# furiosa-ai/eta-inversion

Hardware: AMD Instinct MI355X
Metric: images/sec SD1.5 512^2 50-step etainv+ptp (higher is better)
Workload: dtype bf16; 1 GPU; etainv+ptp, SD1.5-shaped UNet (seeded synthetic weights), 512x512 (64x64 latents), 50 DDIM steps, 32 image pairs per GPU per step, eta [[0.6, 0], [1, 0.7]], n=10 noise candidates, cfg 7.5/1; images_per_gpu=32, unet_sample_forwards_per_image_reference=300

## Files before the change

### eta-inversion_amd/csrc/attention.hip

```cpp
#include <cstdlib>
#include <type_traits>

#include "common.h"
#include "kernels.h"
#include "self_attn_route.h"

namespace etainv {

template <typename T> struct Frag;
template <> struct Frag<f16> {
  typedef f16x8 v8;
  typedef f16x4 v4;
  static __device__ __forceinline__ f32x4 mfma(v8 a, v8 b, f32x4 c) { return __builtin_amdgcn_mfma_f32_16x16x32_f16(a, b, c, 0, 0, 0); }
};
template <> struct Frag<bf16> {
  typedef bf16x8 v8;
  typedef bf16x4 v4;
  static __device__ __forceinline__ f32x4 mfma(v8 a, v8 b, f32x4 c) { return __builtin_amdgcn_mfma_f32_16x16x32_bf16(a, b, c, 0, 0, 0); }
};

constexpr float NEG_BIG = -1.0e30f;

__device__ __forceinline__ void row_roles(int b, int n_img, int& half, int& role, int& img) {
  half = b / (2 * n_img);
// ... 657 lines not shown
        for (int qb = 0; qb < QB; ++qb) {
          v8 pf[4];
#pragma unroll
          for (int ks = 0; ks < 4; ++ks)
#pragma unroll
            for (int e = 0; e < 8; ++e) pf[ks][e] = (T)__builtin_amdgcn_exp2f(s[qb][ks >> 1][(ks & 1) * 8 + e]);
#pragma unroll
          for (int ks = 0; ks < 4; ++ks)
#pragma unroll
            for (int dt = 0; dt < DT; ++dt) o[qb][dt] = Frag32<T>::mfma(vf[ks][dt], pf[ks], o[qb][dt]);
        }
        if (j + 1 < ntiles) store_p(0, cur ^ 1);
        __syncthreads();
      }
    }

    const int q_base = qblk * QI + wid * (32 * QB);
#pragma unroll
    for (int qb = 0; qb < QB; ++qb) {
      const float l = __shfl(o[qb][GEO::LT][GEO::LI], r + 32 * GEO::LH, 64);
      const float inv = 1.f / l;
      const int query = q_base + qb * 32 + r;
      T* op = out + ((int64_t)b * N + query) * C + hd * D + 4 * h;
#pragma unroll
      for (int g4 = 0; g4 < D / 8; ++g4) {
        const int dt = g4 >> 2, i0 = (g4 & 3) * 4;
        T v[4] = {(T)(o[qb][dt][i0] * inv), (T)(o[qb][dt][i0 + 1] * inv), (T)(o[qb][dt][i0 + 2] * inv), (T)(o[qb][dt][i0 + 3] * inv)};
        *reinterpret_cast<u32x2*>(op + 8 * g4) = *reinterpret_cast<u32x2*>(v);
      }
    }
  }
}

template <typename T, int D, int QT, bool EDIT>
__global__ void __launch_bounds__(256) cross_attn_kernel(const T* __restrict__ q, const T* __restrict__ kv, T* __restrict__ out,
                                                         CrossParams p, int row0) {
  typedef typename Frag<T>::v8 v8;
  typedef typename Frag<T>::v4 v4;
  constexpr int DP = (D + 31) / 32 * 32;
  constexpr int KS = DP / 32;
  constexpr int DT = (D + 15) / 16;
  constexpr int NCH = D / 8;
  constexpr int KC = 96;
  constexpr int KT = 5;
  constexpr int KSTR = DP + 8;
  constexpr int VSTR = KC + 8;
  constexpr int PSTR = 81;

  extern __shared__ __attribute__((aligned(16))) char smem[];
  T* sK = reinterpret_cast<T*>(smem);
  T* sKs = sK + KC * KSTR;
  T* sVt = EDIT ? sKs + KC * KSTR : sKs;
  float* sP = reinterpret_cast<float*>(sVt + DT * 16 * VSTR);
  float* sTab = sP + 4 * QT * 16 * PSTR;

  const int tid = threadIdx.x, lane = tid & 63, wid = tid >> 6;
  const int fr = lane & 15, q4 = lane >> 4;
  int bx = blockIdx.x, gxn = gridDim.x, h = blockIdx.y, bz = blockIdx.z;
  if (p.xcd_gx > 0) {
    const int lin = blockIdx.x, xcd = lin & 7, t = lin >> 3;
    h = t % p.heads;
    const int c = (t / p.heads) * 8 + xcd;
    gxn = p.xcd_gx;
    bx = c % gxn;
    bz = c / gxn;
  }
  const int b = row0 + bz;
  const int N = p.N, C = p.heads * D, C2 = 2 * C;

  int img = 0, role = -1, is_cond = 0;
  if (p.layout == 2) {
    int half;
    row_roles(b + p.first_row, p.n_img, half, role, img);
    is_cond = half;
  } else if (p.layout == 1) {
    img = b % p.n_img;
    is_cond = (p.rows == p.n_img) ? 1 : (b / p.n_img);
    role = 0;
  } else if (p.layout == 3) {
    const int g = b / p.n_img;
    img = b % p.n_img;
    is_cond = g >= 1;
    role = g == 1 ? 1 : 0;
  }
  const bool do_edit = EDIT && p.edit && p.layout == 2 && is_cond && role == 1;
  const bool do_store = p.map_layer >= 0 && is_cond;
  const int bs = b - p.n_img;

  for (int idx = tid; idx < KC * (KSTR / 8); idx += 256) {
    const int key = idx / (KSTR / 8), ch = idx % (KSTR / 8);
    u32x4 a = {0u, 0u, 0u, 0u}, s = {0u, 0u, 0u, 0u};
    if (key < p.n_ctx && ch < NCH) {
      a = *reinterpret_cast<const u32x4*>(kv + ((int64_t)b * p.n_ctx + key) * C2 + h * D + ch * 8);
      if (do_edit) s = *reinterpret_cast<const u32x4*>(kv + ((int64_t)bs * p.n_ctx + key) * C2 + h * D + ch * 8);
    }
    *reinterpret_cast<u32x4*>(sK + key * KSTR + ch * 8) = a;
    if (EDIT) *reinterpret_cast<u32x4*>(sKs + key * KSTR + ch * 8) = s;
  }
  for (int idx = tid; idx < KC * NCH; idx += 256) {
    const int key = idx % KC, ch = idx / KC;
    u32x4 c = {0u, 0u, 0u, 0u};
    if (key < p.n_ctx) c = *reinterpret_cast<const u32x4*>(kv + ((int64_t)b * p.n_ctx + key) * C2 + C + h * D + ch * 8);
    const T* e = reinterpret_cast<const T*>(&c);
#pragma unroll
    for (int j = 0; j < 8; ++j) sVt[(ch * 8 + j) * VSTR + key] = e[j];
  }
  if (EDIT && do_edit && tid < p.n_ctx) {
    int mp = p.mapper ? p.mapper[img * 77 + tid] : 0;
    if (mp < 0) mp += p.n_ctx;
    sTab[0 * 80 + tid] = __builtin_bit_cast(float, mp);
    sTab[1 * 80 + tid] = p.alphas ? p.alphas[img * 77 + tid] : 0.f;
    sTab[2 * 80 + tid] = p.equalizer ? p.equalizer[img * 77 + tid] : 1.f;
    sTab[3 * 80 + tid] = p.cross_alpha[img * 77 + tid];
  }
  __syncthreads();

  constexpr bool QPF = D <= 80;
  u32x4 qn[QPF ? QT : 1][QPF ? 2 : 1][QPF ? KS : 1];
  auto load_q = [&](int qb, int qt, int brow, u32x4 (&dst)[QPF ? KS : 1]) __attribute__((always_inline)) {
    int query = qb * (64 * QT) + wid * (16 * QT) + qt * 16 + fr;
    query = query < N ? query : N - 1;
    const T* qp = q + ((int64_t)brow * N + query) * C + h * D;
#pragma unroll
    for (int ks = 0; ks < KS; ++ks) {
      const int d0 = ks * 32 + q4 * 8;
      u32x4 v = {0u, 0u, 0u, 0u};
      if (d0 < D) v = *reinterpret_cast<const u32x4*>(qp + d0);
      dst[ks] = v;
    }
  };
  auto load_block = [&](int qb) __attribute__((always_inline)) {
    if constexpr (QPF) {
#pragma unroll
      for (int qt = 0; qt < QT; ++qt) {
        load_q(qb, qt, b, qn[qt][0]);
        if (do_edit) load_q(qb, qt, bs, qn[qt][1]);
      }
    }
  };
  if (bx * (64 * QT) < N) load_block(bx);
  for (int qb = bx; qb * (64 * QT) < N; qb += gxn) {
  u32x4 qc[QPF ? QT : 1][QPF ? 2 : 1][QPF ? KS : 1];
  if constexpr (QPF) {
#pragma unroll
    for (int qt = 0; qt < QT; ++qt)
#pragma unroll
      for (int e = 0; e < 2; ++e)
#pragma unroll
        for (int ks = 0; ks < KS; ++ks) qc[qt][e][ks] = qn[qt][e][ks];
    if ((qb + gxn) * (64 * QT) < N) load_block(qb + gxn);
// ... 230 lines not shown
    CrossParams pl = p;
    dim3 grid(gx, p.heads, rows);
    if (xcd_heads && (gx * rows) % 8 == 0) {
      pl.xcd_gx = gx;
      grid = dim3(gx * p.heads * rows);
    }
    if (edit)
      hipLaunchKernelGGL((cross_attn_kernel<T, D, QT, true>), grid, dim3(256), lds_edit, s, (const T*)q, (const T*)kv, (T*)out, pl, row0);
    else
      hipLaunchKernelGGL((cross_attn_kernel<T, D, QT, false>), grid, dim3(256), lds_plain, s, (const T*)q, (const T*)kv, (T*)out, pl, row0);
  };
  if (p.edit && p.layout == 2) {
    const int edit0 = 3 * p.n_img - p.first_row;
    launch(false, 0, edit0);
    launch(true, edit0, b - edit0);
  } else {
    launch(false, 0, b);
  }
  ETAINV_LAUNCH_CHECK();
  return 0;
}

int launch_cross_attention_p(const void* q, const void* kv, void* out, int b, int d, const CrossParams& p, int dtype, hipStream_t s) {
  ETAINV_CHECK(q && kv && out && b > 0 && p.N > 0 && p.heads > 0, "bad arguments");
  ETAINV_CHECK(p.n_ctx >= 1 && p.n_ctx <= 77, "n_ctx must be in [1,77]");
  ETAINV_CHECK(d == 40 || d == 80 || d == 160, "head_dim must be 40, 80 or 160");
  ETAINV_CHECK(p.layout >= 0 && p.layout <= 3 && (p.layout == 0 || p.n_img >= 1), "cross-attention: layout 0..3, n_img >= 1");
  ETAINV_CHECK(p.layout != 1 || b == p.n_img || b == 2 * p.n_img, "cross-attention store layout [u, c] x n_img: n_img or 2*n_img rows");
  ETAINV_CHECK(p.layout != 2 || ((p.first_row == 0 || p.first_row == p.n_img) && b + p.first_row == 4 * p.n_img),
               "cross-attention prompt-to-prompt layout: rows [first_row, 4*n_img) of [u_s,u_t,c_s,c_t] x n_img, first_row 0 or n_img");
  ETAINV_CHECK(p.layout != 3 || b == 2 * p.n_img || b == 3 * p.n_img, "cross-attention layout [u_t, c_t, c_s] x n_img: 3*n_img rows, or 2*n_img once the source rows have left");
  ETAINV_CHECK(!p.edit || p.cross_alpha, "cross-attention edit without cross_alpha");
  ETAINV_CHECK(p.map_layer < 0 || (p.maps_acc && p.n_img <= p.n_img_cap), "cross-attention map store: maps_acc missing or n_img > n_img_cap");
  if (dtype == ETAINV_F32) return launch_cross_attention_f32(q, kv, out, b, d, p, s);
  ETAINV_DISPATCH_HALF(dtype, T, switch (d) {
    case 40: return launch_cross_t<T, 40>(q, kv, out, b, p, s);
    case 80: return launch_cross_t<T, 80>(q, kv, out, b, p, s);
    case 160: return launch_cross_t<T, 160>(q, kv, out, b, p, s);
    default: ETAINV_FAIL("head_dim must be 40, 80 or 160");
  });
  return 0;
}

}
```

### eta-inversion_amd/csrc/engine.cpp

```cpp
#include <cmath>
#include <cstring>
#include <functional>
#include <memory>
#include <string>
#include <unordered_map>
#include <vector>

#include "common.h"
#include "kernels.h"

namespace etainv {

static thread_local std::string g_err;
void set_error(const std::string& msg) { g_err = msg; }

struct ProfRec { int cls; double work, bytes; hipEvent_t a, b; };
static bool g_prof_on = false;
static std::vector<ProfRec> g_prof;
static std::vector<std::pair<hipEvent_t, hipEvent_t>> g_prof_pool;
static size_t g_prof_used = 0;
static bool g_prof_paused = false;
bool prof_enabled() { return g_prof_on && !g_prof_paused; }
void prof_pause(bool on) { g_prof_paused = on; }
void prof_begin(int cls, double work, hipStream_t s, double bytes) {
// ... 52 lines not shown

struct etainv_engine {
  etainv_engine_config cfg{};
  int dt = ETAINV_F16;
  size_t esz = 2;
  int L = 64, maxB = 4, max_img = 1;
  static constexpr int kHeads = 8, kCtx = 77, kCtxDim = 768, kGroups = 32, kTemb = 1280, kCh0 = 320;

  std::vector<WeightSlot> slots;
  std::unordered_map<std::string, int> slot_by_name;
  char* warena = nullptr;
  size_t wbytes = 0;
  char* wsarena = nullptr;
  size_t wsbytes = 0;

  void* conv_in_w = nullptr; float* conv_in_b = nullptr;
  void* conv_out_w = nullptr; float* conv_out_b = nullptr;
  Norm norm_out;
  Lin time1, time2, tproj;
  int tproj_total = 0;
  std::vector<ResBlock> res;
  std::vector<TBlock> tb;
  Lin down_conv[3], up_conv[3];

  void *skip[12] = {}, *tmp[3] = {}, *gnbuf = nullptr, *h1 = nullptr, *scbuf = nullptr;
  void *hsA = nullptr, *hsB = nullptr, *lnbuf = nullptr, *qkvbuf = nullptr, *attnbuf = nullptr, *qbuf = nullptr, *kvbuf = nullptr,
       *ffbuf = nullptr, *ctxT = nullptr, *tembuf = nullptr, *temb1 = nullptr, *temb2 = nullptr;
  float *tprojbuf = nullptr, *gn_scratch = nullptr, *maps_acc = nullptr, *lnstat = nullptr, *lnfinal = nullptr;
  size_t maps_bytes = 0;
  int map_div = 4, map_layers = 5;
  float *maps_alt = nullptr, *maps_cur = nullptr;
  size_t maps_alt_bytes = 0, maps_cur_bytes = 0;
  void* kvcache[16] = {};
  bool ctx_cache_on = false;
  const void* ctx_cached = nullptr;
  int ctx_rows = 0, ctx_io = -1;
  void* gn_bufs[16] = {};
  float* gn_part[16] = {};
  float* gn_final = nullptr;
  bool gn_fused = true;
  bool ln_fused = true;
  bool ln_folded = false;
  std::vector<hipStream_t> upload_streams;
  uint64_t ctx_gen = 0, ctx_gen_cached = 0;

  struct Tap { std::string name; int side = 1, channels = 0; void* dst = nullptr; int rows = 0; };
  std::vector<Tap> taps;
  int tap_index(const std::string& name) const {
    for (size_t i = 0; i < taps.size(); ++i)
      if (taps[i].name == name) return (int)i;
    return -1;
  }
  size_t tap_bytes(const Tap& t, int rows) const { return (size_t)rows * t.side * t.side * t.channels * esz; }

  long long qkv_hm_launches = 0;
  bool qkv_hm = true;
};

namespace {

struct ArenaPlan {
  size_t off = 0;
  size_t take(size_t bytes) {
    size_t o = off;
    off += (bytes + 255) & ~(size_t)255;
    return o;
// ... 230 lines not shown
    if (i < 3) {
      side *= 2;
      add(b + ".upsamplers.0", side, rev[i]);
    }
  }
  add("conv_norm_out", L, ch[0]);
}

int build_workspace(etainv_engine* e) {
  ArenaPlan plan;
  std::vector<std::function<void(char*)>> fix;
  auto want = [&](void** field, size_t bytes) {
    size_t off = plan.take(bytes);
    fix.push_back([field, off](char* base) { *field = base + off; });
  };
  const size_t B = (size_t)e->maxB, L = (size_t)e->L, esz = e->esz;
  const size_t hw[4] = {L * L, (L / 2) * (L / 2), (L / 4) * (L / 4), (L / 8) * (L / 8)};
  const size_t skip_el[12] = {hw[0] * 320, hw[0] * 320, hw[0] * 320, hw[1] * 320,  hw[1] * 640,  hw[1] * 640,
                              hw[2] * 640, hw[2] * 1280, hw[2] * 1280, hw[3] * 1280, hw[3] * 1280, hw[3] * 1280};
  for (int i = 0; i < 12; ++i) want(&e->skip[i], B * skip_el[i] * esz);
  const size_t hmax = hw[0] * 320;
  for (int i = 0; i < 3; ++i) want(&e->tmp[i], B * hw[0] * 640 * esz);
  want(&e->gnbuf, B * hw[0] * 960 * esz);
  want(&e->h1, B * hmax * esz);
  want(&e->scbuf, B * hmax * esz);
  want(&e->hsA, B * hmax * esz);
  want(&e->hsB, B * hmax * esz);
  want(&e->lnbuf, B * hmax * esz);
  want(&e->qkvbuf, B * hmax * 3 * esz);
  want(&e->attnbuf, B * hmax * esz);
  want(&e->qbuf, B * hmax * esz);
  want(&e->kvbuf, B * 77 * 2 * 1280 * esz);
  for (size_t i = 0; i < e->tb.size() && i < 16; ++i) want(&e->kvcache[i], B * 77 * 2 * (size_t)e->tb[i].c * esz);
  want(&e->ffbuf, B * hmax * 4 * esz);
  want(&e->ctxT, B * 77 * 768 * esz);
  want(&e->tembuf, B * 320 * esz);
  want(&e->temb1, B * 1280 * esz);
  want(&e->temb2, B * 1280 * esz);
  want(reinterpret_cast<void**>(&e->tprojbuf), B * (size_t)e->tproj_total * 4);
  want(reinterpret_cast<void**>(&e->gn_scratch), B * (GN_MAX_CHUNKS + 1) * etainv_engine::kGroups * 2 * 4);
  want(reinterpret_cast<void**>(&e->lnstat), B * hmax / 32 * 2 * 4);
  want(reinterpret_cast<void**>(&e->lnfinal), B * hw[0] * 2 * 4);
  for (int i = 0; i < 12; ++i) want(reinterpret_cast<void**>(&e->gn_part[i]), B * skip_el[i] / 16 * 4);
  for (int i = 0; i < 3; ++i) want(reinterpret_cast<void**>(&e->gn_part[12 + i]), B * hw[0] * 640 / 16 * 4);
  want(reinterpret_cast<void**>(&e->gn_part[15]), B * hmax / 16 * 4);
  want(reinterpret_cast<void**>(&e->gn_final), B * (etainv_engine::kGroups * 2 + 2 * 2560) * 4);
  const size_t res = L / 4;
  e->maps_bytes = (size_t)5 * e->max_img * 2 * etainv_engine::kHeads * res * res * 77 * 4;
  want(reinterpret_cast<void**>(&e->maps_acc), e->maps_bytes);
  e->wsbytes = plan.off;
  ETAINV_HIP(hipMalloc(reinterpret_cast<void**>(&e->wsarena), e->wsbytes));
  for (auto& f : fix) f(e->wsarena);
  for (int i = 0; i < 12; ++i) e->gn_bufs[i] = e->skip[i];
  for (int i = 0; i < 3; ++i) e->gn_bufs[12 + i] = e->tmp[i];
  e->gn_bufs[15] = e->h1;
  ETAINV_HIP(hipMemset(e->maps_acc, 0, e->maps_bytes));
  e->maps_cur = e->maps_acc;
  e->maps_cur_bytes = e->maps_bytes;
  return 0;
}

struct Fwd {
  etainv_engine* e;
  hipStream_t s;
  int rows;
  const etainv_attn_ctrl* ctrl;
// ... 130 lines not shown
    if (groupnorm(x, nullptr, c, 0, t.gn, hw, 1e-6f, 0)) return 1;
    if (run_ln_out(linear(e->gnbuf, t.proj_in, e->hsA, M))) return 1;
    int head_major = 0;
    IGemmParams qkv;
    if (ln_consumer(qkv, e->hsA, t.ln1, t.s_qkv, t.c_qkv, t.qkv, e->qkvbuf, M)) return 1;
    if (fold && e->qkv_hm && self_attn_prescaled_hm_ok(d, e->dt)) {
      IGemmParams hm = qkv;
      hm.hm_heads = etainv_engine::kHeads;
      hm.hm_dim = d;
      hm.hm_tokens = hw;
      if (igemm_hm_ok(hm, e->dt)) {
        head_major = 1;
        ++e->qkv_hm_launches;
        qkv = hm;
      }
    }
    if (run(qkv)) return 1;
    if (launch_self_attention_mode(e->qkvbuf, e->attnbuf, rows, hw, etainv_engine::kHeads, d, mode, n_img, e->dt, s, self_attn_prescaled_hm_ok(d, e->dt),
                                   ctrl ? (ctrl->src_exit_block ? -1 : ctrl->first_row) : 0, head_major)) return 1;
    IGemmParams o1 = linear(e->attnbuf, t.out1, e->hsB, M);
    o1.residual = e->hsA;
    if (run_ln_out(o1)) return 1;
    if (self_rows != all_rows) {
      const size_t off = (size_t)M * c * e->esz, Mn = (size_t)(all_rows - self_rows) * hw;
      ETAINV_HIP(hipMemcpyAsync(reinterpret_cast<char*>(e->hsB) + off, e->hsB, Mn * c * e->esz, hipMemcpyDeviceToDevice, s));
      if (fold) ETAINV_HIP(hipMemcpyAsync(e->lnfinal + (size_t)M * 2, e->lnfinal, Mn * 2 * sizeof(float), hipMemcpyDeviceToDevice, s));
      rows = all_rows;
      M = rows * hw;
    }
    IGemmParams q;
    if (ln_consumer(q, e->hsB, t.ln2, t.s_q, t.c_q, t.q, e->qbuf, M) || run(q)) return 1;
    void* kvb = e->kvcache[blk];
    if (!kv_reuse && run(linear(e->ctxT, t.kv, kvb, ctx_rows * etainv_engine::kCtx))) return 1;
    CrossParams cp;
    cp.N = hw;
    cp.heads = etainv_engine::kHeads;
    cp.n_ctx = etainv_engine::kCtx;
    cp.scale_log2 = (1.0f / std::sqrt((float)d)) * 1.4426950408889634f;
    cp.rows = rows;
    cp.n_img_cap = e->max_img;
    cp.maps_acc = e->maps_cur;
    cross_params_from_ctrl(cp, ctrl);
    if (cp.layout) {
      const int res = e->L / e->map_div;
      if (ctrl->store_maps && hw == res * res) {
        static const int layer_of_block[3][16] = {{-1, -1, 0, 1, -1, -1, -1, -1, -1, -1, 2, 3, 4, -1, -1, -1},
                                                  {-1, -1, -1, -1, 0, 1, -1, 2, 3, 4, -1, -1, -1, -1, -1, -1},
                                                  {-1, -1, -1, -1, -1, -1, 0, -1, -1, -1, -1, -1, -1, -1, -1, -1}};
        cp.map_layer = layer_of_block[e->map_div == 2 ? 0 : e->map_div == 4 ? 1 : 2][blk];
      }
    }
    if (launch_cross_attention_p(e->qbuf, kvb, e->attnbuf, rows, d, cp, e->dt, s)) return 1;
    IGemmParams o2 = linear(e->attnbuf, t.out2, e->hsA, M);
    o2.residual = e->hsB;
    if (run_ln_out(o2)) return 1;
    IGemmParams ff1;
    if (ln_consumer(ff1, e->hsA, t.ln3, t.s_ff1, t.c_ff1, t.ff1, e->ffbuf, M)) return 1;
    ff1.geglu = 1;
    if (run(ff1)) return 1;
    IGemmParams ff2 = linear(e->ffbuf, t.ff2, e->hsB, M);
    ff2.residual = e->hsA;
    if (run(ff2)) return 1;
    IGemmParams po = linear(e->hsB, t.proj_out, out, M);
    po.residual = x;
    return run(po, true);
  }
};

void* pick_tmp(etainv_engine* e, const void* a, const void* b) {
  for (int i = 0; i < 3; ++i)
    if (e->tmp[i] != a && e->tmp[i] != b) return e->tmp[i];
  return nullptr;
}

}

extern "C" int etainv_abi_version(void) { return ETAINV_ABI_VERSION; }
extern "C" const char* etainv_last_error(void) { return g_err.c_str(); }

extern "C" int etainv_engine_create(const etainv_engine_config* cfg, etainv_engine_t** out) {
  ETAINV_CHECK(cfg && out, "null argument");
  ETAINV_CHECK(cfg->compute_dtype == ETAINV_F16 || cfg->compute_dtype == ETAINV_BF16 || cfg->compute_dtype == ETAINV_F32, "compute_dtype must be f16, bf16 or f32");
  ETAINV_CHECK(cfg->latent_size >= 8 && cfg->latent_size % 8 == 0 && cfg->latent_size <= 128, "latent_size must be a multiple of 8 in [8,128]");
  ETAINV_CHECK(cfg->max_unet_batch >= 1 && cfg->max_img >= 1, "batch sizes must be positive");
  int ndev = 0;
  ETAINV_HIP(hipGetDeviceCount(&ndev));
  ETAINV_CHECK(ndev > 0, "no HIP device visible: the etainv engine has no CPU fallback");
  auto* e = new etainv_engine();
  e->cfg = *cfg;
  e->dt = cfg->compute_dtype;
  e->L = cfg->latent_size;
  e->maxB = cfg->max_unet_batch;
  e->max_img = cfg->max_img;
  e->esz = e->dt == ETAINV_F32 ? 4 : 2;
  e->ln_fused = !env_on("ETAINV_LN_UNFUSED") && e->dt != ETAINV_F32;
  e->gn_fused = !env_on("ETAINV_GN_UNFUSED") && e->dt != ETAINV_F32;
  e->qkv_hm = env_flag("ETAINV_QKV_HM", true);
  build_taps(e);
  if (build_model(e) || build_workspace(e)) {
    etainv_engine_destroy(e);
    return 1;
  }
  *out = e;
  return 0;
}

extern "C" int etainv_engine_destroy(etainv_engine_t* e) {
  if (!e) return 0;
  if (e->warena) (void)hipFree(e->warena);
  if (e->maps_alt) (void)hipFree(e->maps_alt);
  if (e->wsarena) (void)hipFree(e->wsarena);
  delete e;
  return 0;
}

extern "C" int etainv_engine_num_weights(etainv_engine_t* e) { return e ? (int)e->slots.size() : 0; }

extern "C" int etainv_engine_weight_info(etainv_engine_t* e, int i, char* name, int name_cap, int64_t shape[4], int* ndim) {
  ETAINV_CHECK(e && i >= 0 && i < (int)e->slots.size() && name && shape && ndim, "bad arguments");
  const WeightSlot& s = e->slots[i];
  ETAINV_CHECK((int)s.name.size() + 1 <= name_cap, "name buffer too small");
  std::memcpy(name, s.name.c_str(), s.name.size() + 1);
  for (int k = 0; k < 4; ++k) shape[k] = s.shape[k];
  *ndim = s.ndim;
  return 0;
}

extern "C" int etainv_engine_set_weight(etainv_engine_t* e, const char* name, const float* data, int64_t numel, void* stream) {
  ETAINV_CHECK(e && name && data, "null argument");
// ... 359 lines not shown
```

### eta-inversion_amd/csrc/kernels.h

```cpp
#pragma once
#include "common.h"

namespace etainv {

struct IGemmParams {
  const void* a1 = nullptr;
  const void* a2 = nullptr;
  const void* w = nullptr;
  const float* bias = nullptr;
  const float* rowvec = nullptr;
  int rowvec_stride = 0;
  int out_f32 = 0;
  int out_nchw = 0;
  int pad0 = 0;
  int out_io_dtype = 0;
  const void* residual = nullptr;
  void* out = nullptr;
  const void* zeros = nullptr;
  int debug = 0;
  int hm_heads = 0, hm_dim = 0, hm_tokens = 0, hm_magic = 0;
  unsigned long* stamps = nullptr;
  int M = 0, N = 0;
  int c1 = 0, c2 = 0;
  int H = 1, W = 1;
// ... 76 lines not shown
int launch_groupnorm(const void* x1, const void* x2, int c1, int c2, const float* gamma, const float* beta, void* out,
                     int b, int hw, int groups, float eps, int silu, float* scratch, int dtype, hipStream_t s);
int launch_groupnorm_pre(const void* x1, const void* x2, int c1, int c2, const float* part1, int wm1, const float* part2, int wm2, const float* gamma,
                         const float* beta, void* out, int b, int hw, int groups, float eps, int silu, float* final_stats, int dtype, hipStream_t s);
int launch_gn_finalize(int c1, int c2, const float* part1, int wm1, const float* part2, int wm2, int b, int hw, int groups, float eps, float* final_stats,
                       hipStream_t s, const float* gamma = nullptr, const float* beta = nullptr, float* scsh = nullptr);
int launch_gn_fold(const float* w, const float* gamma, const float* beta, const float* bias, const float* final_stats, int groups, int b, int n, int k,
                   void* wb_out, float* cb_out, int dtype, hipStream_t s);
int launch_layernorm(const void* x, const float* gamma, const float* beta, void* out, int rows, int c, float eps, int dtype,
                     hipStream_t s);
int launch_row_stats(const void* x, float* stat, int rows, int c, float eps, int dtype, hipStream_t s);
int launch_ln_finalize(const float* partials, int P, int cw, float eps, float* stat, int rows, hipStream_t s);

inline bool self_attn_prescaled_hm_ok(int d, int dtype) { return dtype != ETAINV_F32 && (d == 40 || d == 80); }
int launch_self_attention_mode(const void* qkv, void* out, int b, int n, int heads, int d, int mode, int n_img, int dtype,
                               hipStream_t s, int q_prescaled = 0, int first_row = 0, int head_major = 0);
struct CrossParams {
  int N = 0, heads = 8, n_ctx = 77;
  float scale_log2 = 0.f;
  int layout = 0;
  int n_img = 1;
  int rows = 0;
  int first_row = 0;
  int edit = 0;
  int map_layer = -1;
  int n_img_cap = 1;
  const int32_t* mapper = nullptr;
  const float* alphas = nullptr;
  const float* replace_mat = nullptr;
  const float* equalizer = nullptr;
  const float* cross_alpha = nullptr;
  float* maps_acc = nullptr;
  int xcd_gx = 0;
};
inline void cross_params_from_ctrl(CrossParams& cp, const etainv_attn_ctrl* ctrl) {
  if (!ctrl || (ctrl->mode != ETAINV_ATTN_PTP && ctrl->mode != ETAINV_ATTN_STORE)) return;
  const bool ptp = ctrl->mode == ETAINV_ATTN_PTP;
  cp.n_img = ctrl->n_img;
  cp.layout = ptp ? (ctrl->src_exit_block ? 3 : 2) : 1;
  cp.first_row = ptp ? ctrl->first_row : 0;
  if (ptp && (ctrl->mapper || ctrl->replace_mat)) {
    cp.edit = 1;
    cp.mapper = ctrl->mapper;
    cp.alphas = ctrl->alphas;
    cp.replace_mat = ctrl->replace_mat;
    cp.equalizer = ctrl->equalizer;
    cp.cross_alpha = ctrl->cross_alpha;
  }
}
int launch_cross_attention_p(const void* q, const void* kv, void* out, int b, int d, const CrossParams& p, int dtype, hipStream_t s);

int launch_im2col_in(const void* latent, int io_dtype, int n_lat, int rows, int L, void* out, int dtype, hipStream_t s);
int launch_time_embedding(const int64_t* t_host, int rows, int dim, void* out, int dtype, hipStream_t s);
int launch_silu(const void* x, void* out, int64_t n, int dtype, hipStream_t s);
enum PackMode { PK_PLAIN = 0, PK_CONV = 1, PK_GEGLU = 2, PK_CONV_IN_GEMM = 5 };
int launch_pack_ups4(const float* src, void* dst, int cout, int cin, int dtype, hipStream_t s);
int launch_pack_weight(const float* src, void* dst, int64_t rows, int64_t cols, int mode, int taps, int dtype, hipStream_t s, float scale = 1.0f,
                       const float* colscale = nullptr);
int launch_ln_fold(const float* w_src, const float* gamma, const float* beta, const float* bias_packed, int64_t rows, int64_t cols, int mode, float scale,
                   void* w_dst, float* s_dst, float* c_dst, int dtype, hipStream_t s);
int launch_cast_f32(const void* src, int src_dtype, void* dst, int dst_dtype, int64_t n, hipStream_t s);
int launch_rows_broadcast(void* x, int rows, int n_src, int64_t row_elems, int dtype, hipStream_t s);

int launch_prox_guidance(const float* eps_u, const float* eps_c, float g, int mode, int use_rank, int rank_lo, float rank_w, float thr_fixed,
                         float* eps_out, const float* x, float a_from, float a_to, float* x_out, float* thr_out, int n_groups, int rows_per_group,
                         int l, hipStream_t s);

// ... 11 lines not shown
```

### eta-inversion_amd/csrc/ops_capi.cpp

```cpp
#include <cmath>

#include "common.h"
#include "kernels.h"

using namespace etainv;

extern "C" int etainv_op_gemm(const void* a, const void* w, const void* bias, const void* residual, void* out, int m, int n, int k,
                              int geglu, int dtype, void* stream) {
  IGemmParams p = igemm_linear(a, w, (const float*)bias, out, m, n, k);
  p.residual = residual;
  p.geglu = geglu;
  return launch_igemm(p, dtype, (hipStream_t)stream);
}

extern "C" int etainv_op_gemm_ln(const void* a, const void* w_folded, const float* c_vec, const float* s_vec, const float* stat,
                                 const void* residual, void* out, float* stat_out, int* stat_p_out, int m, int n, int k, int geglu,
                                 int dtype, void* stream) {
  IGemmParams p = igemm_linear(a, w_folded, c_vec, out, m, n, k);
  p.residual = residual;
  p.geglu = geglu;
  if (stat) {
    p.ln_stat = stat;
    p.ln_s = s_vec;
  }
// ... 92 lines not shown
  p.taps = taps;
  return launch_igemm(p, dtype, (hipStream_t)stream);
}
extern "C" int etainv_op_conv3x3(const void* x_nhwc, const void* x2_nhwc, int c1, int c2, const void* w_okkc, const void* bias,
                                 const float* rowvec, const void* residual, void* out, int b, int h, int wd, int cout, int stride,
                                 int upsample, int taps, int dtype, void* stream) {
  return etainv_op_conv3x3_rv(x_nhwc, x2_nhwc, c1, c2, w_okkc, bias, rowvec, cout, residual, out, b, h, wd, cout, stride, upsample, taps, dtype, stream);
}

extern "C" int etainv_op_groupnorm(const void* x_nhwc, const void* x2_nhwc, int c1, int c2, const float* gamma, const float* beta,
                                   void* out, int b, int hw, int groups, float eps, int silu, float* scratch, int dtype, void* stream) {
  return launch_groupnorm(x_nhwc, x2_nhwc, c1, c2, gamma, beta, out, b, hw, groups, eps, silu, scratch, dtype, (hipStream_t)stream);
}

extern "C" int etainv_op_layernorm(const void* x, const float* gamma, const float* beta, void* out, int rows, int c, float eps, int dtype,
                                   void* stream) {
  return launch_layernorm(x, gamma, beta, out, rows, c, eps, dtype, (hipStream_t)stream);
}

extern "C" int etainv_op_self_attention(const void* qkv, void* out, int b, int n, int heads, int d, int mode, int n_img, int dtype,
                                        void* stream) {
  return launch_self_attention_mode(qkv, out, b, n, heads, d, mode, n_img, dtype, (hipStream_t)stream);
}

extern "C" int etainv_op_self_attention_ex(const void* qkv, void* out, int b, int n, int heads, int d, int mode, int n_img, int q_prescaled, int first_row,
                                           int head_major, int dtype, void* stream) {
  return launch_self_attention_mode(qkv, out, b, n, heads, d, mode, n_img, dtype, (hipStream_t)stream, q_prescaled, first_row, head_major);
}

extern "C" int etainv_op_rows_broadcast(void* x, int rows, int n_src, int64_t row_elems, int dtype, void* stream) {
  return launch_rows_broadcast(x, rows, n_src, row_elems, dtype, (hipStream_t)stream);
}

extern "C" int etainv_op_cross_attention(const void* q, const void* kv, void* out, int b, int n, int heads, int d, int n_ctx,
                                         const etainv_attn_ctrl* ctrl, int map_layer, int n_img_cap, float* maps_acc, int dtype,
                                         void* stream) {
  CrossParams cp;
  cp.N = n;
  cp.heads = heads;
  cp.n_ctx = n_ctx;
  cp.scale_log2 = (1.0f / std::sqrt((float)d)) * 1.4426950408889634f;
  cp.rows = b;
  cp.n_img_cap = n_img_cap;
  cp.maps_acc = maps_acc;
  cross_params_from_ctrl(cp, ctrl);
  if (cp.layout && ctrl->store_maps && map_layer >= 0) cp.map_layer = map_layer;
  return launch_cross_attention_p(q, kv, out, b, d, cp, dtype, (hipStream_t)stream);
}

extern "C" int etainv_op_gemm_f32out(const void* a, const void* w, const float* bias, float* out_f32, int m, int n, int k, int dtype, void* stream) {
  IGemmParams p = igemm_linear(a, w, bias, out_f32, m, n, k);
  p.out_f32 = 1;
  return launch_igemm(p, dtype, (hipStream_t)stream);
}

extern "C" int etainv_op_gn_fold(const float* w, const float* gamma, const float* beta, const float* bias, const float* stats, int groups, int b, int n,
                                 int k, void* wb_out, float* cb_out, int dtype, void* stream) {
  return launch_gn_fold(w, gamma, beta, bias, stats, groups, b, n, k, wb_out, cb_out, dtype, (hipStream_t)stream);
}

extern "C" int etainv_op_gemm_per_image(const void* a, const void* wb, const float* cb, const void* residual, void* out, int b, int hw, int n, int k,
                                        int dtype, void* stream) {
  ETAINV_CHECK(b > 0 && hw > 0, "bad sizes");
  IGemmParams p = igemm_linear(a, wb, cb, out, b * hw, n, k);
  p.residual = residual;
  p.rows_per_batch = hw;
  p.w_batch_stride = (int64_t)n * k;
  p.bias_batch_stride = n;
  return launch_igemm(p, dtype, (hipStream_t)stream);
}
// ... 55 lines not shown
```

### eta-inversion_amd/etainv/_capi.py

```python
import ctypes as C
import os
from pathlib import Path

F32, F16, BF16 = 0, 1, 2
ATTN_PLAIN, ATTN_STORE, ATTN_PTP, ATTN_MASA, ATTN_PNP = 0, 1, 2, 3, 4

_LIB_PATH = Path(__file__).resolve().parent / "lib" / "libetainv_hip.so"


class EtainvError(RuntimeError):
    pass


class EngineConfig(C.Structure):
    _fields_ = [("compute_dtype", C.c_int), ("max_unet_batch", C.c_int), ("latent_size", C.c_int), ("max_img", C.c_int),
                ("reserved", C.c_int * 4)]


class AttnCtrl(C.Structure):
    _fields_ = [("mode", C.c_int), ("n_img", C.c_int), ("store_maps", C.c_int),
                ("mapper", C.c_void_p), ("alphas", C.c_void_p), ("replace_mat", C.c_void_p), ("equalizer", C.c_void_p),
                ("cross_alpha", C.c_void_p),
                ("self_replace_active", C.c_int), ("self_max_tokens", C.c_int),
                ("masa_active", C.c_int), ("masa_first_block", C.c_int), ("first_row", C.c_int), ("src_exit_block", C.c_int), ("pnp_qk_active", C.c_int), ("pnp_conv_active", C.c_int)]
# ... 45 lines not shown
    "etainv_engine_tap_rows": [_p, _i],
    "etainv_engine_workspace_bytes": [_p],
    "etainv_engine_weight_bytes": [_p],
    "etainv_prof_enable": [_i],
    "etainv_prof_reset": [],
    "etainv_prof_read": [_i, C.POINTER(C.c_double), C.POINTER(C.c_double), C.POINTER(_i64)],
    "etainv_prof_records": [_i, C.POINTER(C.c_double), C.POINTER(C.c_double), _i64, C.POINTER(_i64)],
    "etainv_prof_records_ex": [_i, C.POINTER(C.c_double), C.POINTER(C.c_double), C.POINTER(C.c_double), _i64, C.POINTER(_i64)],
    "etainv_prof_split": [_i, C.c_double, C.POINTER(C.c_double), C.POINTER(_i64)],
    "etainv_op_gemm": [_p, _p, _p, _p, _p, _i, _i, _i, _i, _i, _p],
    "etainv_op_gemm_ln": [_p, _p, _p, _p, _p, _p, _p, _p, C.POINTER(_i), _i, _i, _i, _i, _i, _p],
    "etainv_op_gemm_ln_hm": [_p, _p, _p, _p, _p, _p, _i, _i, _i, _i, _i, _i, C.POINTER(_i), _i, _p],
    "etainv_engine_cache_context": [_p, _i],
    "etainv_engine_context_generation": [_p, C.c_uint64],
    "etainv_op_gemm_gnstat": [_p, _p, _p, _p, _p, _p, C.POINTER(_i), _i, _i, _i, _i, _i, _p],
    "etainv_op_conv3x3_gnstat": [_p, _p, _p, _p, _p, _p, _p, C.POINTER(_i), _i, _i, _i, _i, _i, _i, _p],
    "etainv_op_groupnorm_pre": [_p, _p, _i, _i, _p, _i, _p, _i, _p, _p, _p, _i, _i, _i, _f, _i, _p, _i, _p],
    "etainv_op_ln_fold": [_p, _p, _p, _p, _i, _i, _i, _f, _p, _p, _p, _i, _p],
    "etainv_op_row_stats": [_p, _p, _i, _i, _f, _i, _p],
    "etainv_op_ln_finalize": [_p, _i, _i, _f, _p, _i, _p],
    "etainv_op_pack_ups4": [_p, _p, _i, _i, _i, _p],
    "etainv_op_conv3x3": [_p, _p, _i, _i, _p, _p, _p, _p, _p, _i, _i, _i, _i, _i, _i, _i, _i, _p],
    "etainv_op_conv3x3_ex": [_p, _p, _p, _p, _p, _i, _i, _i, _i, _i, _i, _i, _i, _i, _i, _i, _p],
    "etainv_op_im2col3x3": [_p, _i, _i, _i, _i, _i, _p, _p, _i, _p],
    "etainv_op_row_softmax": [_p, _i, _i, _f, _i, _p],
    "etainv_op_quick_gelu": [_p, _p, _i64, _i, _p],
    "etainv_op_embed": [_p, _p, _p, _i, _i, _i, _p, _i, _p],
    "etainv_op_causal_attention": [_p, _p, _i, _i, _i, _i, _i, _p],
    "etainv_op_groupnorm": [_p, _p, _i, _i, _p, _p, _p, _i, _i, _i, _f, _i, _p, _i, _p],
    "etainv_op_layernorm": [_p, _p, _p, _p, _i, _i, _f, _i, _p],
    "etainv_op_self_attention": [_p, _p, _i, _i, _i, _i, _i, _i, _i, _p],
    "etainv_op_self_attention_ex": [_p, _p, _i, _i, _i, _i, _i, _i, _i, _i, _i, _i, _p],
    "etainv_op_cross_attention": [_p, _p, _p, _i, _i, _i, _i, _i, C.POINTER(AttnCtrl), _i, _i, _p, _i, _p],
    "etainv_op_word_maps": [_p, _i, _i, _i, _i, _i, _i, _p, _i, _i, _p, _i, _f, _p],
    "etainv_op_local_blend": [_p, _i, _i, _i, _i, _i, _p, _i, _p, _f, _p],
    "etainv_op_word_maps_ex": [_p, _i, _i, _i, _i, _i, _i, _p, _i, _i, _i, C.c_uint, _p, _i, _f, _p],
    "etainv_op_time_embedding": [C.POINTER(_i64), _i, _i, _p, _i, _p],
    "etainv_op_silu": [_p, _p, _i64, _i, _p],
    "etainv_op_cast": [_p, _i, _p, _i, _i64, _p],
    "etainv_op_im2col_in": [_p, _i, _i, _i, _i, _p, _i, _p],
    "etainv_op_pack_weight": [_p, _p, _i64, _i64, _i, _i, _f, _p, _i, _p],
    "etainv_op_gemm_f32out": [_p, _p, _p, _p, _i, _i, _i, _i, _p],
    "etainv_op_conv3x3_rv": [_p, _p, _i, _i, _p, _p, _p, _i, _p, _p, _i, _i, _i, _i, _i, _i, _i, _i, _p],
    "etainv_op_gn_fold": [_p, _p, _p, _p, _p, _i, _i, _i, _i, _p, _p, _i, _p],
    "etainv_op_gemm_per_image": [_p, _p, _p, _p, _p, _i, _i, _i, _i, _i, _p],
    "etainv_op_rows_broadcast": [_p, _i, _i, _i64, _i, _p],
    "etainv_op_last_igemm_plan": [C.POINTER(_i), _i],
    "etainv_op_igemm_route_name": [_i],
}
_RESTYPES = {"etainv_last_error": C.c_char_p, "etainv_op_igemm_route_name": C.c_char_p,"etainv_engine_workspace_bytes": _i64, "etainv_image_metrics_workspace_bytes": _i64, "etainv_engine_weight_bytes": _i64}

_lib = None


def lib_path() -> Path:
    return Path(os.environ.get("ETAINV_LIB", _LIB_PATH))


def load():
    global _lib
    if _lib is None:
        path = lib_path()
        if not path.exists():
            raise EtainvError(f"{path} not found: build it with eta-inversion_amd/csrc/build.sh (no CPU fallback exists)")
        lib = C.CDLL(str(path))
        for name, args in SIGNATURES.items():
            fn = getattr(lib, name)
            fn.argtypes = args
            fn.restype = _RESTYPES.get(name, C.c_int)
        _lib = lib
    return _lib


def check(status: int):
    if status != 0:
        raise EtainvError(load().etainv_last_error().decode())


def dtype_code(dt) -> int:
    import torch
    return {torch.float32: F32, torch.float16: F16, torch.bfloat16: BF16}[dt]


# ... 11 lines not shown
```

### include/etainv.h

```cpp
#ifndef ETAINV_H
#define ETAINV_H
#include <stdint.h>
#ifdef __cplusplus
extern "C" {
#endif

#define ETAINV_ABI_VERSION 1
#define ETAINV_MAX_WORDS 77

enum etainv_dtype { ETAINV_F32 = 0, ETAINV_F16 = 1, ETAINV_BF16 = 2 };

int etainv_abi_version(void);
const char* etainv_last_error(void);


int etainv_cfg_combine(const void* eps_u, const void* eps_c, float g, void* out, int64_t n,
                       int io_dtype, void* stream);

int etainv_ddim_step(const void* x, const void* eps, float a_from, float a_to, void* out, int64_t n,
                     int io_dtype, void* stream);

int etainv_ddim_eta_step(const void* x, const void* eps, float eta, const void* eta_mask, int n_mask, const void* noise,
                         float a_t, float a_p, float var, int rows, int c, int hw, void* out, int io_dtype, void* stream);

// ... 133 lines not shown
int etainv_op_gemm_gnstat(const void* a, const void* w, const float* bias, const void* residual, void* out, float* part, int* wm_out, int m,
                          int n, int k, int rows_per_image, int dtype, void* stream);
int etainv_op_conv3x3_gnstat(const void* x_nhwc, const void* w_okkc, const float* bias, const float* rowvec, const void* residual, void* out,
                             float* part, int* wm_out, int b, int h, int wd, int cin, int cout, int dtype, void* stream);
int etainv_op_groupnorm_pre(const void* x1, const void* x2, int c1, int c2, const float* part1, int wm1, const float* part2, int wm2,
                            const float* gamma, const float* beta, void* out, int b, int hw, int groups, float eps, int silu,
                            float* final_stats, int dtype, void* stream);
int etainv_op_pack_ups4(const float* w_oc33, void* dst, int cout, int cin, int dtype, void* stream);
int etainv_op_conv3x3(const void* x_nhwc, const void* x2_nhwc, int c1, int c2, const void* w_okkc, const void* bias,
                      const float* rowvec, const void* residual, void* out, int b, int h, int wd, int cout,
                      int stride, int upsample, int taps, int dtype, void* stream);
int etainv_op_conv3x3_ex(const void* x_nhwc, const void* w_okkc, const void* bias, const void* residual, void* out, int b, int h,
                         int wd, int cin, int cout, int stride, int upsample, int pad0, int out_nchw, int out_io_dtype, int dtype,
                         void* stream);
int etainv_op_im2col3x3(const void* x_nchw, int io_dtype, int cin, int h, int w, int rows, const float* premix, void* out,
                        int dtype, void* stream);
int etainv_op_row_softmax(void* x, int rows, int n, float scale, int dtype, void* stream);
int etainv_op_quick_gelu(const void* x, void* out, int64_t n, int dtype, void* stream);
int etainv_op_embed(const int64_t* ids, const void* tok, const void* pos, int b, int n_pos, int d, void* out, int dtype,
                    void* stream);
int etainv_op_causal_attention(const void* qkv, void* out, int b, int n, int heads, int d, int dtype, void* stream);
int etainv_op_groupnorm(const void* x_nhwc, const void* x2_nhwc, int c1, int c2, const float* gamma,
                        const float* beta, void* out, int b, int hw, int groups, float eps, int silu,
                        float* scratch, int dtype, void* stream);
int etainv_op_layernorm(const void* x, const float* gamma, const float* beta, void* out, int rows, int c,
                        float eps, int dtype, void* stream);
int etainv_op_self_attention(const void* qkv, void* out, int b, int n, int heads, int d, int mode, int n_img,
                             int dtype, void* stream);
int etainv_op_self_attention_ex(const void* qkv, void* out, int b, int n, int heads, int d, int mode, int n_img,
                                int q_prescaled, int first_row, int head_major, int dtype, void* stream);
int etainv_op_cross_attention(const void* q, const void* kv, void* out, int b, int n, int heads, int d,
                              int n_ctx, const etainv_attn_ctrl* ctrl, int map_layer, int n_img_cap,
                              float* maps_acc, int dtype, void* stream);
int etainv_op_word_maps(const float* maps_acc, int n_layers, int n_img_cap, int heads, int res, int L, int n_img,
                        const int32_t* tokens, int n_tok, int steps_done, float* out, int accumulate, float scale,
                        void* stream);
int etainv_op_local_blend(const float* maps_acc, int n_layers, int n_img_cap, int heads, int res, int L, float* x,
                          int n_img, const float* blend_alpha, float thres, void* stream);

int etainv_op_word_maps_ex(const float* maps_acc, int n_layers, int n_img_cap, int heads, int res, int L, int n_img,
                           const int32_t* tokens, int n_tok, int steps_done, int row_sel, unsigned layer_mask, float* out,
                           int accumulate, float scale, void* stream);
int etainv_op_time_embedding(const int64_t* t_host, int rows, int dim, void* out, int dtype, void* stream);
int etainv_op_silu(const void* x, void* out, int64_t n, int dtype, void* stream);
int etainv_op_cast(const void* src, int src_dtype, void* dst, int dst_dtype, int64_t n, void* stream);
int etainv_op_im2col_in(const void* latent, int io_dtype, int n_lat, int rows, int l, void* out, int dtype, void* stream);
int etainv_op_pack_weight(const float* src, void* dst, int64_t rows, int64_t cols, int mode, int taps, float scale, const float* colscale,
                          int dtype, void* stream);
int etainv_op_rows_broadcast(void* x, int rows, int n_src, int64_t row_elems, int dtype, void* stream);
int etainv_op_gemm_f32out(const void* a, const void* w, const float* bias, float* out_f32, int m, int n, int k, int dtype, void* stream);
int etainv_op_conv3x3_rv(const void* x_nhwc, const void* x2_nhwc, int c1, int c2, const void* w_okkc, const void* bias,
                         const float* rowvec, int rowvec_stride, const void* residual, void* out, int b, int h, int wd, int cout,
                         int stride, int upsample, int taps, int dtype, void* stream);
int etainv_op_gn_fold(const float* w, const float* gamma, const float* beta, const float* bias, const float* stats, int groups, int b, int n,
                      int k, void* wb_out, float* cb_out, int dtype, void* stream);
int etainv_op_gemm_per_image(const void* a, const void* wb, const float* cb, const void* residual, void* out, int b, int hw, int n, int k,
                             int dtype, void* stream);
int etainv_op_last_igemm_plan(int* out, int n);
const char* etainv_op_igemm_route_name(int route);

#ifdef __cplusplus
}
#endif
#endif
```

Measured before the change: 5.836 images/s.

## Precompute padded shared-memory K/V images for cross-attention once per context

Adds a kernel that writes each head's cross-attention K block and transposed V block into global memory, already padded in the exact shared-memory layout. It runs once whenever the context K/V projection is recomputed. Each cross-attention block then fills shared memory with straight vectorised copies instead of scattered transposing stores, and this cost is shared across the many query blocks of a head. It also turns on Q prefetch for the D=160 non-edit kernel. The price is extra workspace per transformer block and one extra kernel launch per K/V recompute.

New measurement: 5.846 images/s, median of 6. No clear change (+0.2%).

```diff
diff --git a/eta-inversion_amd/csrc/attention.hip b/eta-inversion_amd/csrc/attention.hip
--- a/eta-inversion_amd/csrc/attention.hip
+++ b/eta-inversion_amd/csrc/attention.hip
@@ -713,6 +713,36 @@
   }
 }
 
+template <typename T, int D>
+__global__ void __launch_bounds__(256) cross_kv_image_kernel(const T* __restrict__ kv, T* __restrict__ image, int heads, int n_ctx) {
+  constexpr int DP = (D + 31) / 32 * 32, DT = (D + 15) / 16, NCH = D / 8;
+  constexpr int KC = 96, KSTR = DP + 8, VSTR = KC + 8;
+  constexpr int K16 = KC * KSTR / 8, V16 = DT * 16 * VSTR / 8;
+  __shared__ __attribute__((aligned(16))) T sVt[DT * 16 * VSTR];
+  const int tid = threadIdx.x, h = blockIdx.x, b = blockIdx.y;
+  const int C = heads * D, C2 = 2 * C;
+  const T* src = kv + (int64_t)b * n_ctx * C2 + h * D;
+  u32x4* dst = reinterpret_cast<u32x4*>(image + ((int64_t)b * heads + h) * (int64_t)(K16 + V16) * 8);
+  const u32x4 zero = {0u, 0u, 0u, 0u};
+  for (int idx = tid; idx < V16; idx += 256) reinterpret_cast<u32x4*>(sVt)[idx] = zero;
+  for (int idx = tid; idx < K16; idx += 256) {
+    const int key = idx / (KSTR / 8), ch = idx % (KSTR / 8);
+    u32x4 a = zero;
+    if (key < n_ctx && ch < NCH) a = *reinterpret_cast<const u32x4*>(src + (int64_t)key * C2 + ch * 8);
+    dst[idx] = a;
+  }
+  __syncthreads();
+  for (int idx = tid; idx < n_ctx * NCH; idx += 256) {
+    const int key = idx / NCH, ch = idx % NCH;
+    const u32x4 c = *reinterpret_cast<const u32x4*>(src + (int64_t)key * C2 + C + ch * 8);
+    const T* e = reinterpret_cast<const T*>(&c);
+#pragma unroll
+    for (int j = 0; j < 8; ++j) sVt[(ch * 8 + j) * VSTR + key] = e[j];
+  }
+  __syncthreads();
+  for (int idx = tid; idx < V16; idx += 256) dst[K16 + idx] = reinterpret_cast<const u32x4*>(sVt)[idx];
+}
+
 template <typename T, int D, int QT, bool EDIT>
 __global__ void __launch_bounds__(256) cross_attn_kernel(const T* __restrict__ q, const T* __restrict__ kv, T* __restrict__ out,
                                                          CrossParams p, int row0) {
@@ -768,6 +798,19 @@
   const bool do_store = p.map_layer >= 0 && is_cond;
   const int bs = b - p.n_img;
 
+  if (p.kv_image) {
+    constexpr int K16 = KC * KSTR / 8, V16 = DT * 16 * VSTR / 8;
+    const u32x4* im = reinterpret_cast<const u32x4*>(p.kv_image) + ((int64_t)b * p.heads + h) * (K16 + V16);
+#pragma unroll 4
+    for (int idx = tid; idx < K16; idx += 256) reinterpret_cast<u32x4*>(sK)[idx] = im[idx];
+#pragma unroll 4
+    for (int idx = tid; idx < V16; idx += 256) reinterpret_cast<u32x4*>(sVt)[idx] = im[K16 + idx];
+    if constexpr (EDIT) {
+      const u32x4* ims = reinterpret_cast<const u32x4*>(p.kv_image) + ((int64_t)(do_edit ? bs : b) * p.heads + h) * (K16 + V16);
+#pragma unroll 4
+      for (int idx = tid; idx < K16; idx += 256) reinterpret_cast<u32x4*>(sKs)[idx] = do_edit ? ims[idx] : (u32x4){0u, 0u, 0u, 0u};
+    }
+  } else {
   for (int idx = tid; idx < KC * (KSTR / 8); idx += 256) {
     const int key = idx / (KSTR / 8), ch = idx % (KSTR / 8);
     u32x4 a = {0u, 0u, 0u, 0u}, s = {0u, 0u, 0u, 0u};
@@ -785,6 +828,7 @@
     const T* e = reinterpret_cast<const T*>(&c);
 #pragma unroll
     for (int j = 0; j < 8; ++j) sVt[(ch * 8 + j) * VSTR + key] = e[j];
+  }
   }
   if (EDIT && do_edit && tid < p.n_ctx) {
     int mp = p.mapper ? p.mapper[img * 77 + tid] : 0;
@@ -796,7 +840,7 @@
   }
   __syncthreads();
 
-  constexpr bool QPF = D <= 80;
+  constexpr bool QPF = D <= 80 || !EDIT;
   u32x4 qn[QPF ? QT : 1][QPF ? 2 : 1][QPF ? KS : 1];
   auto load_q = [&](int qb, int qt, int brow, u32x4 (&dst)[QPF ? KS : 1]) __attribute__((always_inline)) {
     int query = qb * (64 * QT) + wid * (16 * QT) + qt * 16 + fr;
@@ -1093,6 +1137,7 @@
   ETAINV_CHECK(p.layout != 3 || b == 2 * p.n_img || b == 3 * p.n_img, "cross-attention layout [u_t, c_t, c_s] x n_img: 3*n_img rows, or 2*n_img once the source rows have left");
   ETAINV_CHECK(!p.edit || p.cross_alpha, "cross-attention edit without cross_alpha");
   ETAINV_CHECK(p.map_layer < 0 || (p.maps_acc && p.n_img <= p.n_img_cap), "cross-attention map store: maps_acc missing or n_img > n_img_cap");
+  ETAINV_CHECK(!p.kv_image || dtype != ETAINV_F32, "cross-attention K / V images: 16-bit kernels only");
   if (dtype == ETAINV_F32) return launch_cross_attention_f32(q, kv, out, b, d, p, s);
   ETAINV_DISPATCH_HALF(dtype, T, switch (d) {
     case 40: return launch_cross_t<T, 40>(q, kv, out, b, p, s);
@@ -1103,4 +1148,24 @@
   return 0;
 }
 
-}
+template <typename T, int D>
+static int launch_cross_kv_image_t(const void* kv, void* image, int rows, int heads, int n_ctx, hipStream_t s) {
+  hipLaunchKernelGGL((cross_kv_image_kernel<T, D>), dim3(heads, rows), dim3(256), 0, s, (const T*)kv, (T*)image, heads, n_ctx);
+  ETAINV_LAUNCH_CHECK();
+  return 0;
+}
+
+int launch_cross_kv_image(const void* kv, void* image, int rows, int heads, int d, int n_ctx, int dtype, hipStream_t s) {
+  ETAINV_CHECK(kv && image && rows > 0 && heads > 0, "bad arguments");
+  ETAINV_CHECK(n_ctx >= 1 && n_ctx <= 77, "n_ctx must be in [1,77]");
+  ETAINV_CHECK(d == 40 || d == 80 || d == 160, "head_dim must be 40, 80 or 160");
+  ETAINV_CHECK(dtype != ETAINV_F32, "cross-attention K / V images: 16-bit kernels only (the fp32 kernel stages from kv)");
+  ETAINV_DISPATCH_HALF(dtype, T, switch (d) {
+    case 40: return launch_cross_kv_image_t<T, 40>(kv, image, rows, heads, n_ctx, s);
+    case 80: return launch_cross_kv_image_t<T, 80>(kv, image, rows, heads, n_ctx, s);
+    default: return launch_cross_kv_image_t<T, 160>(kv, image, rows, heads, n_ctx, s);
+  });
+  return 0;
+}
+
+}
diff --git a/eta-inversion_amd/csrc/engine.cpp b/eta-inversion_amd/csrc/engine.cpp
--- a/eta-inversion_amd/csrc/engine.cpp
+++ b/eta-inversion_amd/csrc/engine.cpp
@@ -108,6 +108,8 @@
   float *maps_alt = nullptr, *maps_cur = nullptr;
   size_t maps_alt_bytes = 0, maps_cur_bytes = 0;
   void* kvcache[16] = {};
+  void* kvimg[16] = {};
+  bool cross_images = true;
   bool ctx_cache_on = false;
   const void* ctx_cached = nullptr;
   int ctx_rows = 0, ctx_io = -1;
@@ -404,6 +406,8 @@
   want(&e->qbuf, B * hmax * esz);
   want(&e->kvbuf, B * 77 * 2 * 1280 * esz);
   for (size_t i = 0; i < e->tb.size() && i < 16; ++i) want(&e->kvcache[i], B * 77 * 2 * (size_t)e->tb[i].c * esz);
+  for (size_t i = 0; e->cross_images && i < e->tb.size() && i < 16; ++i)
+    want(&e->kvimg[i], B * etainv_engine::kHeads * cross_kv_image_bytes(e->tb[i].c / etainv_engine::kHeads));
   want(&e->ffbuf, B * hmax * 4 * esz);
   want(&e->ctxT, B * 77 * 768 * esz);
   want(&e->tembuf, B * 320 * esz);
@@ -600,7 +604,9 @@
     if (ln_consumer(q, e->hsB, t.ln2, t.s_q, t.c_q, t.q, e->qbuf, M) || run(q)) return 1;
     void* kvb = e->kvcache[blk];
     if (!kv_reuse && run(linear(e->ctxT, t.kv, kvb, ctx_rows * etainv_engine::kCtx))) return 1;
+    if (!kv_reuse && e->cross_images && launch_cross_kv_image(kvb, e->kvimg[blk], ctx_rows, etainv_engine::kHeads, d, etainv_engine::kCtx, e->dt, s)) return 1;
     CrossParams cp;
+    cp.kv_image = e->cross_images ? e->kvimg[blk] : nullptr;
     cp.N = hw;
     cp.heads = etainv_engine::kHeads;
     cp.n_ctx = etainv_engine::kCtx;
@@ -663,6 +669,7 @@
   e->esz = e->dt == ETAINV_F32 ? 4 : 2;
   e->ln_fused = !env_on("ETAINV_LN_UNFUSED") && e->dt != ETAINV_F32;
   e->gn_fused = !env_on("ETAINV_GN_UNFUSED") && e->dt != ETAINV_F32;
+  e->cross_images = env_flag("ETAINV_CROSS_IMAGES", true) && e->dt != ETAINV_F32;
   e->qkv_hm = env_flag("ETAINV_QKV_HM", true);
   build_taps(e);
   if (build_model(e) || build_workspace(e)) {
diff --git a/eta-inversion_amd/csrc/kernels.h b/eta-inversion_amd/csrc/kernels.h
--- a/eta-inversion_amd/csrc/kernels.h
+++ b/eta-inversion_amd/csrc/kernels.h
@@ -132,7 +132,12 @@
   const float* cross_alpha = nullptr;
   float* maps_acc = nullptr;
   int xcd_gx = 0;
+  const void* kv_image = nullptr;
 };
+constexpr size_t cross_kv_image_bytes(int d) {
+  return ((size_t)96 * ((d + 31) / 32 * 32 + 8) + (size_t)((d + 15) / 16) * 16 * (96 + 8)) * 2;
+}
+int launch_cross_kv_image(const void* kv, void* image, int rows, int heads, int d, int n_ctx, int dtype, hipStream_t s);
 inline void cross_params_from_ctrl(CrossParams& cp, const etainv_attn_ctrl* ctrl) {
   if (!ctrl || (ctrl->mode != ETAINV_ATTN_PTP && ctrl->mode != ETAINV_ATTN_STORE)) return;
   const bool ptp = ctrl->mode == ETAINV_ATTN_PTP;
diff --git a/eta-inversion_amd/csrc/ops_capi.cpp b/eta-inversion_amd/csrc/ops_capi.cpp
--- a/eta-inversion_amd/csrc/ops_capi.cpp
+++ b/eta-inversion_amd/csrc/ops_capi.cpp
@@ -148,10 +148,26 @@
   return launch_rows_broadcast(x, rows, n_src, row_elems, dtype, (hipStream_t)stream);
 }
 
+extern "C" int64_t etainv_cross_kv_image_bytes(int rows, int heads, int d) {
+  if (rows <= 0 || heads <= 0 || (d != 40 && d != 80 && d != 160)) return 0;
+  return (int64_t)rows * heads * (int64_t)cross_kv_image_bytes(d);
+}
+
+extern "C" int etainv_op_cross_kv_image(const void* kv, void* image, int b, int heads, int d, int n_ctx, int dtype, void* stream) {
+  return launch_cross_kv_image(kv, image, b, heads, d, n_ctx, dtype, (hipStream_t)stream);
+}
+
 extern "C" int etainv_op_cross_attention(const void* q, const void* kv, void* out, int b, int n, int heads, int d, int n_ctx,
                                          const etainv_attn_ctrl* ctrl, int map_layer, int n_img_cap, float* maps_acc, int dtype,
                                          void* stream) {
+  return etainv_op_cross_attention_img(q, kv, nullptr, out, b, n, heads, d, n_ctx, ctrl, map_layer, n_img_cap, maps_acc, dtype, stream);
+}
+
+extern "C" int etainv_op_cross_attention_img(const void* q, const void* kv, const void* kv_image, void* out, int b, int n, int heads, int d, int n_ctx,
+                                             const etainv_attn_ctrl* ctrl, int map_layer, int n_img_cap, float* maps_acc, int dtype,
+                                             void* stream) {
   CrossParams cp;
+  cp.kv_image = kv_image;
   cp.N = n;
   cp.heads = heads;
   cp.n_ctx = n_ctx;
diff --git a/eta-inversion_amd/etainv/_capi.py b/eta-inversion_amd/etainv/_capi.py
--- a/eta-inversion_amd/etainv/_capi.py
+++ b/eta-inversion_amd/etainv/_capi.py
@@ -101,6 +101,9 @@
     "etainv_op_self_attention": [_p, _p, _i, _i, _i, _i, _i, _i, _i, _p],
     "etainv_op_self_attention_ex": [_p, _p, _i, _i, _i, _i, _i, _i, _i, _i, _i, _i, _p],
     "etainv_op_cross_attention": [_p, _p, _p, _i, _i, _i, _i, _i, C.POINTER(AttnCtrl), _i, _i, _p, _i, _p],
+    "etainv_cross_kv_image_bytes": [_i, _i, _i],
+    "etainv_op_cross_kv_image": [_p, _p, _i, _i, _i, _i, _i, _p],
+    "etainv_op_cross_attention_img": [_p, _p, _p, _p, _i, _i, _i, _i, _i, C.POINTER(AttnCtrl), _i, _i, _p, _i, _p],
     "etainv_op_word_maps": [_p, _i, _i, _i, _i, _i, _i, _p, _i, _i, _p, _i, _f, _p],
     "etainv_op_local_blend": [_p, _i, _i, _i, _i, _i, _p, _i, _p, _f, _p],
     "etainv_op_word_maps_ex": [_p, _i, _i, _i, _i, _i, _i, _p, _i, _i, _i, C.c_uint, _p, _i, _f, _p],
@@ -117,7 +120,8 @@
     "etainv_op_last_igemm_plan": [C.POINTER(_i), _i],
     "etainv_op_igemm_route_name": [_i],
 }
-_RESTYPES = {"etainv_last_error": C.c_char_p, "etainv_op_igemm_route_name": C.c_char_p,"etainv_engine_workspace_bytes": _i64, "etainv_image_metrics_workspace_bytes": _i64, "etainv_engine_weight_bytes": _i64}
+_RESTYPES = {"etainv_last_error": C.c_char_p, "etainv_op_igemm_route_name": C.c_char_p,"etainv_engine_workspace_bytes": _i64, "etainv_image_metrics_workspace_bytes": _i64, "etainv_engine_weight_bytes": _i64,
+             "etainv_cross_kv_image_bytes": _i64}
 
 _lib = None
 
diff --git a/include/etainv.h b/include/etainv.h
--- a/include/etainv.h
+++ b/include/etainv.h
@@ -189,6 +189,11 @@
 int etainv_op_cross_attention(const void* q, const void* kv, void* out, int b, int n, int heads, int d,
                               int n_ctx, const etainv_attn_ctrl* ctrl, int map_layer, int n_img_cap,
                               float* maps_acc, int dtype, void* stream);
+int64_t etainv_cross_kv_image_bytes(int rows, int heads, int d);
+int etainv_op_cross_kv_image(const void* kv, void* image, int b, int heads, int d, int n_ctx, int dtype, void* stream);
+int etainv_op_cross_attention_img(const void* q, const void* kv, const void* kv_image, void* out, int b, int n, int heads, int d,
+                                  int n_ctx, const etainv_attn_ctrl* ctrl, int map_layer, int n_img_cap,
+                                  float* maps_acc, int dtype, void* stream);
 int etainv_op_word_maps(const float* maps_acc, int n_layers, int n_img_cap, int heads, int res, int L, int n_img,
                         const int32_t* tokens, int n_tok, int steps_done, float* out, int accumulate, float scale,
                         void* stream);
```
